# dhruvmetha/rapid-locomotion-rl

Hardware: AMD Instinct MI355X
Metric: env-steps/sec, 4096 Mini Cheetah envs, 1/2/4/8 MI355X; PPO iters/sec (higher is better)
Workload: dtype f32; 1 GPU; 4096 Mini Cheetah envs flat terrain (4096 per GPU), PPO teacher policy (BASELINE configs[1]); envs_per_gpu=4096, global_envs=4096, global_batch_env_steps_per_iter=98304, parallelism=dp1, world_size=1, policy=ActorCritic 42/18/630->12, random init; teacher PPO + student adaptation update

## Files before the change

### rapid-locomotion-rl_amd/csrc/lrl_gemm.h

```cpp
#pragma once
#include <stdint.h>

#ifdef __HIPCC__
#define LRL_GHD __host__ __device__
#else
#define LRL_GHD
#endif

namespace lrl {

enum GemmEpi : int {
  EPI_STORE = 0,
  EPI_BIAS = 1,
  EPI_BIAS_ELU = 2,
  EPI_DELU = 3,
  EPI_PARTIAL = 4,
  EPI_BIAS_TANH = 5,
  EPI_DTANH = 6,
};

struct GemmP {
  const float* A;
  const float* B;
  float* C;
  const float* bias;
  const float* aux;
  const int64_t* a_rows;
  const int64_t* b_rows;
  float* bias_part;
  int M, N, K;
  int splits, kps;
  int avec, bvec;
  int groups;
  int64_t lda, ldb, ldc, ld_aux;
  int64_t ga, gb, gc, gbias, gaux;
  int64_t part_stride;
  const uint16_t* bpl;
  int64_t bpl_ld, bpl_ps, gbp;
};

struct PlaneJob {
  const float* W;
  int64_t ldw, gsrc;
  int rows, cols, trans, groups;
  uint16_t* dst;
};
constexpr int MAX_PLANE_JOBS = 8;
LRL_GHD inline int plane_kp(const PlaneJob& j) { return ((j.trans ? j.rows : j.cols) + 15) / 16 * 16; }
LRL_GHD inline int plane_n(const PlaneJob& j) { return j.trans ? j.cols : j.rows; }
LRL_GHD inline int64_t plane_elems(const PlaneJob& j) { return 3ll * j.groups * plane_n(j) * plane_kp(j); }
int x6_planes_launch(const PlaneJob* jobs, int n, void* stream);
bool gemm_x6p_enabled();
inline void gemm_use_planes(GemmP& p, const PlaneJob& j) {
  p.bpl = j.dst;
  p.bpl_ld = plane_kp(j);
  p.gbp = (int64_t)plane_n(j) * plane_kp(j);
  p.bpl_ps = p.gbp * j.groups;
}

enum GemmLayout : int { GEMM_NT = 0, GEMM_NN = 2, GEMM_TN = 3 };

int gemm_launch(const GemmP& p, int layout, int epi, int groups, void* stream);

struct GemmJob {
  GemmP p;
  int layout, epi, groups;
};
constexpr int MAX_MULTI_JOBS = 3;
int gemm_launch_multi(const GemmJob* jobs, int n, void* stream);

enum GemmFamily : int {
  FAM_NONE = 0, FAM_X6P = 1, FAM_X6T = 2, FAM_X6 = 3, FAM_X6D = 4, FAM_GLDS = 5, FAM_GLDS32 = 6, FAM_GLDS_TN = 7,
  FAM_THIN16 = 8, FAM_THIN32 = 9, FAM_STAGED = 10,
};
constexpr int gemm_path_id(int family, int bm, int bn, bool interior) {
  return family | (bm << 8) | (bn << 16) | (interior ? 1 << 24 : 0);
}
int gemm_last_path();

int gemm_pick_splits(int M, int N, int K, int groups);

bool gemm_x6_enabled();
constexpr int X6_MIN_M = 64;

#ifdef __HIPCC__
typedef float f32x16 __attribute__((ext_vector_type(16)));
typedef short bf16x8_t __attribute__((ext_vector_type(8)));
constexpr int XBK = 16;

__device__ __forceinline__ float elu_f(float x) { return x > 0.f ? x : expm1f(x); }
__device__ __forceinline__ float tanh_f(float x) { return tanhf(x); }
__host__ __device__ constexpr bool epi_bias(int e) { return e == EPI_BIAS || e == EPI_BIAS_ELU || e == EPI_BIAS_TANH; }
__host__ __device__ constexpr bool epi_aux(int e) { return e == EPI_DELU || e == EPI_DTANH; }
template <int EPI>
__device__ __forceinline__ float epi_apply(float v, float bj, float x) {
  if constexpr (EPI == EPI_BIAS) return v + bj;
  else if constexpr (EPI == EPI_BIAS_ELU) return elu_f(v + bj);
  else if constexpr (EPI == EPI_BIAS_TANH) return tanh_f(v + bj);
  else if constexpr (EPI == EPI_DELU) return x > 0.f ? v : v * (x + 1.f);
  else if constexpr (EPI == EPI_DTANH) return v * (1.f - x * x);
  else return v;
}

__device__ __forceinline__ uint32_t x6_hi_pair(uint32_t u0, uint32_t u1) {
  return __builtin_amdgcn_perm(u1, u0, 0x07060302u);
}
__device__ __forceinline__ void x6_split2(float x0, float x1, uint32_t& h, uint32_t& m, uint32_t& l) {
  uint32_t u0 = __float_as_uint(x0), u1 = __float_as_uint(x1);
  h = x6_hi_pair(u0, u1);
  float r0 = x0 - __uint_as_float(u0 & 0xffff0000u), r1 = x1 - __uint_as_float(u1 & 0xffff0000u);
  u0 = __float_as_uint(r0);
  u1 = __float_as_uint(r1);
  m = x6_hi_pair(u0, u1);
  r0 = r0 - __uint_as_float(u0 & 0xffff0000u);
  r1 = r1 - __uint_as_float(u1 & 0xffff0000u);
  l = x6_hi_pair(__float_as_uint(r0), __float_as_uint(r1));
}
__device__ __forceinline__ int x6_off(int r, int c) { return r * XBK + 8 * (c ^ ((r >> 3) & 1)); }

__device__ __forceinline__ f32x16 x6_mma(const bf16x8_t (&a)[3], const bf16x8_t (&b)[3], f32x16 c) {
  c = __builtin_amdgcn_mfma_f32_32x32x16_bf16(a[2], b[0], c, 0, 0, 0);
  c = __builtin_amdgcn_mfma_f32_32x32x16_bf16(a[1], b[1], c, 0, 0, 0);
  c = __builtin_amdgcn_mfma_f32_32x32x16_bf16(a[0], b[2], c, 0, 0, 0);
  c = __builtin_amdgcn_mfma_f32_32x32x16_bf16(a[1], b[0], c, 0, 0, 0);
  c = __builtin_amdgcn_mfma_f32_32x32x16_bf16(a[0], b[1], c, 0, 0, 0);
  c = __builtin_amdgcn_mfma_f32_32x32x16_bf16(a[0], b[0], c, 0, 0, 0);
  return c;
}
#endif

}
```

### rapid-locomotion-rl_amd/csrc/lrl_ppo.hip

```cpp
#include <hip/hip_runtime.h>
#include <math.h>
#include <stdint.h>
#include <stdlib.h>
#include <string.h>

#include <algorithm>
#include <initializer_list>
#include <mutex>
#include <vector>

#include "../../include/lrl.h"
#include "../../include/lrl_philox.h"
#include "lrl_gemm.h"
#include "lrl_launch.h"

namespace lrl {

constexpr float LOG_SQRT_2PI = 0.91893853320467274178f;
constexpr int HEAD_ROWS = 32;
constexpr int HEAD_THREADS = 256;
constexpr int HEAD_W = 128;
constexpr int MAX_ACT = 16;
constexpr int HEAD_NA = 12;
constexpr int MAX_LAT = 32;

__device__ __forceinline__ float delu(float h) { return h > 0.f ? 1.f : h + 1.f; }

constexpr int PREP_R = 4;
__global__ void ppo_prep_kernel(const float* __restrict__ obs, const int64_t* __restrict__ rows, int B, int no,
                                int xs, float* __restrict__ X) {
  const int64_t i = (int64_t)blockIdx.x * blockDim.x + threadIdx.x;
  const int64_t ng = ((int64_t)B + PREP_R - 1) / PREP_R;
  if (i >= ng * xs) return;
  const int g = (int)(i / xs), c = (int)(i - (int64_t)g * xs);
  int64_t src[PREP_R];
  float v[PREP_R];
#pragma unroll
  for (int u = 0; u < PREP_R; ++u) {
    const int b = g * PREP_R + u;
    src[u] = b < B ? (rows ? rows[b] : (int64_t)b) : -1;
  }
#pragma unroll
  for (int u = 0; u < PREP_R; ++u) v[u] = (c < no && src[u] >= 0) ? obs[src[u] * no + c] : 0.f;
#pragma unroll
  for (int u = 0; u < PREP_R; ++u) {
    const int b = g * PREP_R + u;
    if (b < B) X[(int64_t)b * xs + c] = v[u];
  }
}

inline unsigned prep_blocks(int64_t rows, int xs) {
  return (unsigned)((((rows + PREP_R - 1) / PREP_R) * xs + 255) / 256);
}

struct HeadArgs {
  const float* h3;
  float* dh3;
  const float *w4a, *b4a, *w4c, *b4c, *stdv;
  const float *actions, *old_mu, *old_sigma, *tv, *ret, *adv, *old_logp;
  const int64_t* rows;
  int B, na;
  float clip, ent_coef, vcoef;
  int clipped_value;
  float* part;
  int part_len;
};

__host__ __device__ constexpr int hp_w4a(int) { return 0; }
__host__ __device__ constexpr int hp_b4a(int na) { return na * HEAD_W; }
__host__ __device__ constexpr int hp_w4c(int na) { return na * HEAD_W + na; }
__host__ __device__ constexpr int hp_b4c(int na) { return na * HEAD_W + na + HEAD_W; }
__host__ __device__ constexpr int hp_std(int na) { return na * HEAD_W + na + HEAD_W + 1; }
__host__ __device__ constexpr int hp_kl(int na) { return na * HEAD_W + na + HEAD_W + 1 + na; }
__host__ __device__ constexpr int hp_len(int na) { return hp_kl(na) + 3; }

template <int NA, bool TANH>
__global__ __launch_bounds__(HEAD_THREADS) void ppo_head_kernel(HeadArgs a) {
  constexpr int HP = 2 * HEAD_W + 4;
  constexpr int NAP = (NA + 3) / 4 * 4;
  static_assert(NA <= 16 && HEAD_W % 16 == 0, "float4 rows");
  constexpr int NG = (HEAD_ROWS * NA + HEAD_THREADS - 1) / HEAD_THREADS;
  __shared__ __attribute__((aligned(16))) float H[HEAD_ROWS][HP];
  __shared__ __attribute__((aligned(16))) float W4[NA + 1][HEAD_W];
  __shared__ float MU[HEAD_ROWS][NA + 1];
  __shared__ float VP[HEAD_ROWS][8];
  __shared__ __attribute__((aligned(16))) float LP[HEAD_ROWS][NAP];
  __shared__ float KT[HEAD_ROWS][NA];
  __shared__ float DR[HEAD_ROWS][2];
  __shared__ float SC[HEAD_ROWS][3];
  __shared__ float SD[3][NA];
  __shared__ float GA[3][HEAD_ROWS][NA];
  __shared__ float GR[4][HEAD_ROWS];
  __shared__ int64_t RW[HEAD_ROWS];
  const int t = threadIdx.x;
  const int r0 = blockIdx.x * HEAD_ROWS;
  const int nrows = min(HEAD_ROWS, a.B - r0);
  if (t < HEAD_ROWS) RW[t] = t < nrows ? a.rows[r0 + t] : a.rows[r0];
  if (t < NA) {
    const float sd = a.stdv[t];
    SD[0][t] = sd;
    SD[1][t] = logf(sd);
    SD[2][t] = 1.f / (sd * sd);
  }
  {
    constexpr int NV = HEAD_ROWS * 2 * HEAD_W / 4 / HEAD_THREADS;
    float4 v[NV];
#pragma unroll
    for (int u = 0; u < NV; ++u) {
      const int i = t + u * HEAD_THREADS, r = i / (HEAD_W / 2), c = 4 * (i % (HEAD_W / 2));
      v[u] = r < nrows ? *reinterpret_cast<const float4*>(a.h3 + (int64_t)(r0 + r) * (2 * HEAD_W) + c)
                       : make_float4(0.f, 0.f, 0.f, 0.f);
    }
#pragma unroll
    for (int u = 0; u < NV; ++u) {
      const int i = t + u * HEAD_THREADS, r = i / (HEAD_W / 2), c = 4 * (i % (HEAD_W / 2));
      *reinterpret_cast<float4*>(&H[r][c]) = v[u];
    }
  }
  for (int i = t; i < (NA + 1) * HEAD_W; i += HEAD_THREADS) {
    const int j = i / HEAD_W, k = i - j * HEAD_W;
    W4[j][k] = j < NA ? a.w4a[j * HEAD_W + k] : a.w4c[k];
  }
  __syncthreads();
  float ga[3][NG], gr = 0.f;
#pragma unroll
  for (int u = 0; u < NG; ++u) {
    const int i = t + u * HEAD_THREADS;
    const int r = i / NA, j = i - r * NA;
    const bool ok = i < HEAD_ROWS * NA;
    const int64_t o = RW[ok ? r : 0] * NA + j;
    ga[0][u] = ok ? a.actions[o] : 0.f;
    ga[1][u] = ok ? a.old_mu[o] : 0.f;
    ga[2][u] = ok ? a.old_sigma[o] : 1.f;
  }
  if (t < 4 * HEAD_ROWS) {
    const int q = t / HEAD_ROWS, r = t - q * HEAD_ROWS;
    const float* src = q == 0 ? a.adv : q == 1 ? a.old_logp : q == 2 ? a.tv : a.ret;
    gr = src[RW[r]];
  }
  {
    const int r = t & (HEAD_ROWS - 1), q = t / HEAD_ROWS;
    const float4* hr = reinterpret_cast<const float4*>(&H[r][0]);
    auto dot4 = [](float s, float4 h, float4 w) {
      s = fmaf(h.x, w.x, s);
      s = fmaf(h.y, w.y, s);
      s = fmaf(h.z, w.z, s);
      return fmaf(h.w, w.w, s);
    };
    for (int j = q; j < NA; j += 8) {
      const float4* wr = reinterpret_cast<const float4*>(&W4[j][0]);
      float s = 0.f;
#pragma unroll 8
      for (int k4 = 0; k4 < HEAD_W / 4; ++k4) s = dot4(s, hr[k4], wr[k4]);
      MU[r][j] = s + a.b4a[j];
    }
// ... 714 lines not shown
      else oa_layer<1>(L);
      __syncthreads();
      FA_PROF(5 + l)
    }
    const int64_t so = (int64_t)a.store_row * a.n;
    if (grp == 0) {
      for (int e = t; e < NA * HEAD_W; e += OA_THREADS) HW[e] = w[nt.w4a + e];
      __syncthreads();
      for (int e = t; e < OA_R * NA; e += OA_THREADS) {
        const int r = e & (OA_R - 1), j = e / OA_R;
        float s = 0.f;
        for (int k = 0; k < HEAD_W; ++k) s = fmaf(H3[r * OA_H3P + k], HW[j * HEAD_W + k], s);
        MU[r * 16 + j] = s + w[nt.b4a + j];
      }
      __syncthreads();
      FA_PROF(8)
      for (int i = t; i < nrows * NA; i += OA_THREADS) {
        const int r = i / NA, j = i - r * NA, g = r0 + r;
        const float m = MU[r * 16 + j], sd = w[nt.std_off + j];
        float act;
        MU[r * 16 + j] = act_draw(a.eps, a.row_offset, a.seed, a.counter, g, j, NA, m, sd, act);
        a.actions[(int64_t)g * NA + j] = act;
        if (a.mu) a.mu[(int64_t)g * NA + j] = m;
        if (a.do_store) {
          const int64_t o = (so + g) * NA + j;
          a.store.actions[o] = act;
          a.store.mu[o] = m;
          a.store.sigma[o] = sd;
        }
      }
      __syncthreads();
      if (t < nrows) {
        const int g = r0 + t;
        float lp = 0.f;
        for (int j = 0; j < NA; ++j) lp += MU[t * 16 + j];
        if (a.logp) a.logp[g] = lp;
        if (a.do_store) a.store.logp[so + g] = lp;
      }
    } else {
      for (int e = t; e < HEAD_W; e += OA_THREADS) HW[e] = w[nt.w4c + e];
      __syncthreads();
      for (int e = t; e < OA_R * 16; e += OA_THREADS) {
        const int r = e & (OA_R - 1), q = e / OA_R;
        float s = 0.f;
        for (int k = q * (HEAD_W / 16); k < (q + 1) * (HEAD_W / 16); ++k) s = fmaf(H3[r * OA_H3P + k], HW[k], s);
        VP[r * 16 + q] = s;
      }
      __syncthreads();
      FA_PROF(8)
      if (t < nrows) {
        const int g = r0 + t;
        float vs[16];
#pragma unroll
        for (int q = 0; q < 16; ++q) vs[q] = VP[t * 16 + q];
#pragma unroll
        for (int wd = 8; wd >= 1; wd /= 2)
#pragma unroll
          for (int q = 0; q < wd; ++q) vs[q] = vs[2 * q] + vs[2 * q + 1];
        const float v = vs[0] + w[nt.b4c];
        if (a.values) a.values[g] = v;
        if (a.do_store) a.store.values[so + g] = v;
      }
    }
    FA_PROF(9)
    if (a.do_store) {
      const int64_t b = so + r0;
      if (grp == 0) copy_rows<OA_THREADS>(a.obs + (int64_t)r0 * no, no, a.store.obs + b * no, no, nrows, no, t);
      else copy_rows<OA_THREADS>(a.priv + (int64_t)r0 * np, np, a.store.priv + b * np, np, nrows, np, t);
      if (a.hist && a.store.hist) {
        const int hd = a.store.hist_dim, ld = a.store.hist_ld > hd ? a.store.hist_ld : hd;
        const int h0 = grp * (OA_R / 2), hn = min(nrows, h0 + OA_R / 2) - h0;
        if (hn > 0) copy_rows<OA_THREADS>(a.hist + (int64_t)(r0 + h0) * hd, hd, a.store.hist + (b + h0) * ld, ld, hn, hd, t);
      }
    }
    FA_PROF(10)
  }
}

struct AdaptHeadArgs {
  const float* hd2;
  int ldh;
  const float* tgt;
  int ldt;
  float* dhd2;
  const float *w, *b;
  int B, H, L;
  float* part;
  int part_len;
};

template <int CH, int CL>
__global__ __launch_bounds__(HEAD_THREADS) void adapt_head_kernel(AdaptHeadArgs a) {
  const int H = CH ? CH : a.H, L = CL ? CL : a.L;
  __shared__ float HS[HEAD_ROWS][MAX_LAT + 1];
  __shared__ float DP[HEAD_ROWS][MAX_LAT + 1];
  __shared__ float WS[MAX_LAT][MAX_LAT + 1];
  __shared__ float TG[HEAD_ROWS][MAX_LAT + 1];
  __shared__ float ERR[HEAD_ROWS];
  const int t = threadIdx.x;
  const int r0 = blockIdx.x * HEAD_ROWS;
  const int nrows = min(HEAD_ROWS, a.B - r0);
  for (int i = t; i < HEAD_ROWS * H; i += HEAD_THREADS) {
    const int r = i / H, c = i - r * H;
    HS[r][c] = r < nrows ? a.hd2[(int64_t)(r0 + r) * a.ldh + c] : 0.f;
  }
  for (int i = t; i < L * H; i += HEAD_THREADS) WS[i / H][i % H] = a.w[i];
  for (int i = t; i < HEAD_ROWS * L; i += HEAD_THREADS) {
    const int r = i / L, j = i - r * L;
    TG[r][j] = r < nrows ? a.tgt[(int64_t)(r0 + r) * a.ldt + j] : 0.f;
  }
  __syncthreads();
  const float scale = 2.f / ((float)a.B * (float)L);
  for (int i = t; i < HEAD_ROWS * L; i += HEAD_THREADS) {
    const int r = i / L, j = i - r * L;
    float d = 0.f;
    if (r < nrows) {
      float s = 0.f;
      for (int k = 0; k < H; ++k) s = fmaf(HS[r][k], WS[j][k], s);
      const float pred = s + a.b[j];
      d = pred - TG[r][j];
    }
    TG[r][j] = d * d;
    DP[r][j] = scale * d;
  }
  __syncthreads();
  if (t < HEAD_ROWS) {
    float e = 0.f;
    for (int j = 0; j < L; ++j) e += TG[t][j];
    ERR[t] = e;
  }
  __syncthreads();
  float* P = a.part + (int64_t)blockIdx.x * a.part_len;
  for (int i = t; i < nrows * H; i += HEAD_THREADS) {
    const int r = i / H, k = i - r * H;
    float s = 0.f;
    for (int j = 0; j < L; ++j) s = fmaf(DP[r][j], WS[j][k], s);
    a.dhd2[(int64_t)(r0 + r) * a.ldh + k] = s * delu(HS[r][k]);
  }
  const int nr = CH ? HEAD_ROWS : nrows;
  for (int i = t; i < L * H; i += HEAD_THREADS) {
    const int j = i / H, k = i - j * H;
    float s = 0.f;
    for (int r = 0; r < nr; ++r) s = fmaf(DP[r][j], HS[r][k], s);
    P[i] = s;
  }
  if (t < L) {
    float s = 0.f;
    for (int r = 0; r < nr; ++r) s += DP[r][t];
    P[L * H + t] = s;
  } else if (t == 64) {
    float s = 0.f;
    for (int r = 0; r < nr; ++r) s += ERR[r];
    P[L * H + L] = s;
  }
}

struct Seg {
  const float* src;
  float* dst;
  int64_t len, stride;
  int parts;
  float scale;
  int lpg;
  int blk0, nblk;
};
constexpr int MAX_SEGS = 24;
struct SegList {
  Seg s[MAX_SEGS];
  int n;
};

__global__ __launch_bounds__(256) void seg_reduce_kernel(SegList L) {
  int si = 0;
  while (si + 1 < L.n && (int)blockIdx.x >= L.s[si + 1].blk0) ++si;
  const Seg& sg = L.s[si];
  const int lpg = sg.lpg, pg = 1 << lpg, E = 256 >> lpg;
  const int e = threadIdx.x & (E - 1), g = threadIdx.x >> (8 - lpg);
  __shared__ float red[256];
  for (int64_t base = (int64_t)(blockIdx.x - sg.blk0) * E; base < sg.len; base += (int64_t)sg.nblk * E) {
    const int64_t i = base + e;
    float acc = 0.f;
    if (i < sg.len) {
      const float* p = sg.src + i;
      int q = g;
      for (; q + 7 * pg < sg.parts; q += 8 * pg) {
        float v[8];
#pragma unroll
        for (int u = 0; u < 8; ++u) v[u] = __builtin_nontemporal_load(p + (int64_t)(q + u * pg) * sg.stride);
#pragma unroll
        for (int u = 0; u < 8; ++u) acc += v[u];
      }
      for (; q < sg.parts; q += pg) acc += p[(int64_t)q * sg.stride];
    }
    if (pg == 1) {
      if (i < sg.len) sg.dst[i] = acc * sg.scale;
      continue;
    }
    red[threadIdx.x] = acc;
    __syncthreads();
    if (g == 0 && i < sg.len) {
      float t = 0.f;
      for (int k = 0; k < pg; ++k) t += red[k * E + e];
      sg.dst[i] = t * sg.scale;
    }
    __syncthreads();
  }
}

constexpr int NORM_BLOCKS = 256;
__global__ void sumsq_kernel(const float* __restrict__ g, int64_t n, double* __restrict__ part) {
  double s = 0.0;
  for (int64_t i = (int64_t)blockIdx.x * blockDim.x + threadIdx.x; i < n; i += (int64_t)gridDim.x * blockDim.x) {
    const double x = g[i];
    s += x * x;
  }
  for (int off = 32; off > 0; off >>= 1) s += __shfl_down(s, off, 64);
  __shared__ double red[4];
  if ((threadIdx.x & 63) == 0) red[threadIdx.x >> 6] = s;
  __syncthreads();
  if (threadIdx.x == 0) part[blockIdx.x] = (red[0] + red[1]) + (red[2] + red[3]);
}

__global__ void ppo_finalize_kernel(const double* __restrict__ part, int nparts, const float* __restrict__ kl_slot,
                                    float grad_scale, float max_norm, float desired_kl, int adaptive, double bc1,
                                    float inv_B, lrl_ppo_ctrl* ctrl) {
  __shared__ double red[64];
  double s = 0.0;
  for (int i = threadIdx.x; i < nparts; i += 64) s += part[i];
  red[threadIdx.x] = s;
  __syncthreads();
  if (threadIdx.x != 0) return;
  double tot = 0.0;
  for (int i = 0; i < 64; ++i) tot += red[i];
  const float total_norm = (float)sqrt(tot) * grad_scale;
  float clip = max_norm / (total_norm + 1e-6f);
  clip = fminf(clip, 1.f);
  double lr = ctrl->lr;
  const float kl = kl_slot[0] * grad_scale;
  if (adaptive) {
    const double k = (double)kl;
    if (k > (double)desired_kl * 2.0) lr = fmax(1e-5, lr / 1.5);
    else if (k < (double)desired_kl / 2.0 && k > 0.0) lr = fmin(1e-2, lr * 1.5);
  }
  ctrl->lr = lr;
  ctrl->mb[3] = kl;
  ctrl->clip_scale = clip;
  ctrl->total_norm = total_norm;
  ctrl->step_size = (float)(lr / bc1);
  ctrl->loss_sum[0] += (double)ctrl->mb[0];
  ctrl->loss_sum[1] += (double)ctrl->mb[1];
}

__global__ void adam_kernel(float* __restrict__ p, const float* __restrict__ g, float* __restrict__ m,
                            float* __restrict__ v, int64_t n, float grad_scale, const lrl_ppo_ctrl* __restrict__ ctrl,
                            float step_size_host, float one_minus_b1, float b2, float one_minus_b2, float bc2_sqrt,
                            float eps, lrl_ppo_ctrl* acc_ctrl) {
  const float clip = ctrl ? ctrl->clip_scale : 1.f;
  const float step = ctrl ? ctrl->step_size : step_size_host;
  for (int64_t i = (int64_t)blockIdx.x * blockDim.x + threadIdx.x; i < n; i += (int64_t)gridDim.x * blockDim.x) {
    float gi = g[i] * grad_scale;
    gi = gi * clip;
    float mi = m[i];
    mi = mi + one_minus_b1 * (gi - mi);
    float vi = v[i] * b2;
    vi = vi + one_minus_b2 * gi * gi;
    m[i] = mi;
    v[i] = vi;
    const float denom = sqrtf(vi) / bc2_sqrt + eps;
    p[i] = p[i] + (-step) * (mi / denom);
  }
  if (acc_ctrl && blockIdx.x == 0 && threadIdx.x == 0) acc_ctrl->loss_sum[2] += (double)acc_ctrl->mb[2];
}

__global__ void pad_cols_kernel(const float* __restrict__ W, int rows, int h, int hp, float* __restrict__ Wp) {
  const int64_t n = (int64_t)rows * hp;
  for (int64_t i = (int64_t)blockIdx.x * blockDim.x + threadIdx.x; i < n; i += (int64_t)gridDim.x * blockDim.x) {
    const int r = (int)(i / hp), c = (int)(i - (int64_t)r * hp);
    Wp[i] = c < h ? W[(int64_t)r * h + c] : 0.f;
  }
}


static int xs_of(const lrl_ppo_net& n) {
  if (n.plain) return (n.num_obs + 15) / 16 * 16;
  const int nx = n.num_obs + n.latent;
  return nx <= 64 ? 64 : (nx + 15) / 16 * 16;
}
constexpr int LATS = 32;
constexpr int HD2S = 32;
static int hist_pad(int h) { return (h + 15) / 16 * 16; }

enum MainPlane { PL_W1, PL_W2, PL_W3, PL_E2, PL_W2T, PL_W3T, PL_E2T, PL_MAIN };
constexpr int PL_FWD = PL_E2 + 1;
enum AdaptPlane { PL_D1, PL_AE2, PL_D2T, PL_ADAPT };

struct Layer {
  int64_t w, b;
  int out, in;
  int64_t ldw;
  int kf;
  int groups;
  int fwd, bwd;
};
static Layer layer(int64_t w, int64_t b, int out, int in, int groups = 1, int fwd = -1, int bwd = -1) {
  return Layer{w, b, out, in, in, in, groups, fwd, bwd};
}
// ... 556 lines not shown
  return hipGetLastError() == hipSuccess ? 0 : lrl_set_error(LRL_E_HIP, "lrl_ppo_act: launch failed");
}

extern "C" int64_t lrl_ppo_act_student_workspace_bytes(const lrl_ppo_net* net, int32_t n) {
  if (check_net(net) || net->plain || n <= 0) return -1;
  return make_student_plan(*net, n, nullptr).bytes;
}

extern "C" int32_t lrl_ppo_act_student(const lrl_ppo_net* net, const float* params, const float* obs,
                                       const float* hist, int32_t hist_ld, int32_t n, float* mean, float* latent,
                                       void* workspace, void* stream) {
  if (int rc = check_net(net)) return rc;
  if (net->plain) return lrl_set_error(LRL_E_INVALID, "lrl_ppo_act_student: a plain net has no adaptation module");
  if (!params || !obs || !hist || !mean || !workspace || n <= 0)
    return lrl_set_error(LRL_E_INVALID, "lrl_ppo_act_student: null argument or n <= 0");
  const lrl_ppo_net& nt = *net;
  const int hld = hist_ld ? hist_ld : nt.num_hist;
  if (hld < nt.num_hist) return lrl_set_error(LRL_E_INVALID, "lrl_ppo_act_student: hist_ld < num_hist");
  Plan P = make_student_plan(nt, n, static_cast<char*>(workspace));
  hipStream_t st = static_cast<hipStream_t>(stream);
  G g{st, params, n};
  const Net L = layers_of(nt, true);
  const Buf lat = cols_from(P.xa, nt.num_obs);
  prep_x(nt, obs, nullptr, n, P.xa, st);
  adaptation_l1_forward(g, L.ad[0], In{hist, hld}, nullptr, P);
  g.forward(L.ad[1], P.hd1, nullptr, P.hd2, true);
  g.forward(L.ad[2], P.hd2, nullptr, lat, false);
  body_forward(g, L.body, P);
  g.forward(L.mean, P.h3, nullptr, Buf{mean, nt.num_actions}, false);
  if (g.rc) return lrl_set_error(g.rc, "lrl_ppo_act_student: GEMM launch failed");
  if (latent &&
      hipMemcpy2DAsync(latent, (size_t)nt.latent * 4, lat.p, (size_t)lat.ld * 4, (size_t)nt.latent * 4, n,
                       hipMemcpyDeviceToDevice, st) != hipSuccess)
    return lrl_set_error(LRL_E_HIP, "lrl_ppo_act_student: latent copy failed");
  return hipGetLastError() == hipSuccess ? 0 : lrl_set_error(LRL_E_HIP, "lrl_ppo_act_student: launch failed");
}

extern "C" int64_t lrl_ppo_workspace_bytes(const lrl_ppo_net* net, int32_t batch) {
  if (check_net(net) || batch <= 0) return -1;
  return make_plan(*net, batch, nullptr).bytes;
}

extern "C" int32_t lrl_ppo_forward_backward(const lrl_ppo_net* net, const float* params, float* grads,
                                            const lrl_ppo_batch* bt, const lrl_ppo_hparams* hp, void* workspace,
                                            lrl_ppo_ctrl* ctrl, void* stream) {
  if (int rc = check_net(net)) return rc;
  if (!bt || !hp || !params || !grads || !workspace || !ctrl || bt->batch <= 0)
    return lrl_set_error(LRL_E_INVALID, "lrl_ppo_forward_backward: null argument");
  const lrl_ppo_net& n = *net;
  const int B = bt->batch;
  const bool full = !n.plain;
  Plan P = make_plan(n, B, static_cast<char*>(workspace));
  hipStream_t st = static_cast<hipStream_t>(stream);
  G g{st, params, B, P.part, P.part + P.part_floats};
  g.tanh_act = n.plain;
  const Net net_l = layers_of(n);
  const Layer(&enc)[3] = net_l.enc;
  const Layer(&body)[3] = net_l.body;
  PlaneJob pj[PL_MAIN];
  if (full) {
    main_plane_jobs(n, params, P.wpl, pj);
    if (int rc = split_planes(pj, PL_MAIN, gemm_x6p_enabled(), st))
      return lrl_set_error(rc, "lrl_ppo_forward_backward: planes launch failed");
    g.with(pj);
  }
  const In priv{bt->priv, n.num_priv};
  prep_x(n, bt->obs, bt->rows, B, P.xa, st);
  if (full) encoder_forward(g, enc, priv, bt->rows, P, cols_from(P.xa, n.num_obs));
  body_forward(g, body, P);
  if (g.rc) return lrl_set_error(g.rc, "lrl_ppo_forward_backward: forward GEMM launch failed");
  SegList L{};
  launch_loss_head(n, params, grads, bt, hp, ctrl, P, g.part, L, st);
  g.backward_data(body[2], P.dh3, P.dh2, P.h2);
  g.backward_data(body[1], P.dh2, P.dh1, P.h1);
  if (full) g.backward_data(net_l.dlat, P.dh1, P.dlat, In{});
  enum { DWE3, DHE2, DWE2, DHE1, DWE1, DW3, DW2, DW1, NJOBS };
  GemmJob jobs[NJOBS];
  const int first = full ? 0 : DW3;
  g.collect(jobs, first, NJOBS);
  if (full) {
    g.weight_grad(enc[2], P.dlat, P.he2, nullptr, grads, L);
    g.backward_data(enc[2], P.dlat, P.dhe2, P.he2);
    g.weight_grad(enc[1], P.dhe2, P.he1, nullptr, grads, L);
    g.backward_data(enc[1], P.dhe2, P.dhe1, P.he1);
    g.weight_grad(enc[0], P.dhe1, priv, bt->rows, grads, L);
  }
  g.weight_grad(body[2], P.dh3, P.h2, nullptr, grads, L);
  g.weight_grad(body[1], P.dh2, P.h1, nullptr, grads, L);
  g.weight_grad(body[0], P.dh1, P.xa, nullptr, grads, L);
  int rc = g.rc ? g.rc : (g.njobs == NJOBS ? 0 : LRL_E_INVALID);
  if (rc) return lrl_set_error(rc, "lrl_ppo_forward_backward: backward GEMM launch failed");
  struct Set { int n, i[MAX_MULTI_JOBS]; };
  Set sets[NJOBS];
  int ns = 0;
  const int mode = full ? bwd_multi_mode() : 0;
  if (mode == 0) {
    for (int i = first; i < NJOBS; ++i) sets[ns++] = Set{1, {i}};
  } else if (g_timer.on) {
    sets[ns++] = Set{3, {DWE3, DHE2, DW3}};
    sets[ns++] = Set{2, {DWE2, DHE1}};
    sets[ns++] = Set{1, {DW2}};
    sets[ns++] = Set{2, {DWE1, DW1}};
  } else {
    static const int hosts[3][3] = {{DW3, DW1, DW2}, {DW3, DW2, DW1}, {DW2, DW1, DW3}};
    const int* host = hosts[mode - 1];
    sets[ns++] = Set{3, {DWE3, DHE2, host[0]}};
    sets[ns++] = Set{3, {DWE2, DHE1, host[1]}};
    sets[ns++] = Set{2, {DWE1, host[2]}};
  }
  Fork* fk = mode == 0 && full ? fork_for_device(st) : nullptr;
  if (fk && (hipEventRecord(fk->go, st) != hipSuccess || hipStreamWaitEvent(fk->st, fk->go, 0) != hipSuccess))
    return lrl_set_error(LRL_E_HIP, "lrl_ppo_forward_backward: stream fork failed");
  for (int s = 0; s < ns && !rc; ++s) {
    const int lead = sets[s].i[0];
    const bool timed = full && sets[s].n == 1 && lead == DW2;
    if (timed) timer_begin(st);
    rc = launch_jobs(jobs, sets[s].i, sets[s].n, fk && lead < DW3 ? fk->st : st);
    if (timed) timer_end(st);
    if (fk && lead == DWE1 && hipEventRecord(fk->done, fk->st) != hipSuccess)
      return lrl_set_error(LRL_E_HIP, "lrl_ppo_forward_backward: stream fork failed");
  }
  if (fk && hipStreamWaitEvent(st, fk->done, 0) != hipSuccess)
    return lrl_set_error(LRL_E_HIP, "lrl_ppo_forward_backward: stream join failed");
  if (rc) return lrl_set_error(rc, "lrl_ppo_forward_backward: backward GEMM launch failed");
  launch_seg(L, st);
  return hipGetLastError() == hipSuccess ? 0 : lrl_set_error(LRL_E_HIP, "lrl_ppo_forward_backward: launch failed");
}

extern "C" int32_t lrl_ppo_optimizer_step(const lrl_ppo_net* net, float* params, const float* grads, float* exp_avg,
                                          float* exp_avg_sq, int64_t step, float grad_scale,
                                          const lrl_ppo_hparams* hp, void* workspace, lrl_ppo_ctrl* ctrl,
                                          void* stream) {
  if (int rc = check_net(net)) return rc;
  if (!params || !grads || !exp_avg || !exp_avg_sq || !hp || !workspace || !ctrl || step < 1)
    return lrl_set_error(LRL_E_INVALID, "lrl_ppo_optimizer_step: bad argument");
  const lrl_ppo_net& n = *net;
  hipStream_t st = static_cast<hipStream_t>(stream);
  double* norm_part = static_cast<double*>(workspace);
  const int64_t len = n.main_end - n.main_begin;
  hipLaunchKernelGGL(sumsq_kernel, dim3(NORM_BLOCKS), dim3(256), 0, st, grads + n.main_begin, len, norm_part);
  const double bc1 = 1.0 - pow((double)hp->beta1, (double)step);
  const double bc2 = 1.0 - pow((double)hp->beta2, (double)step);
  hipLaunchKernelGGL(ppo_finalize_kernel, dim3(1), dim3(64), 0, st, norm_part, NORM_BLOCKS,
                     grads + n.kl_slot, grad_scale, hp->max_grad_norm, hp->desired_kl, hp->adaptive_schedule, bc1,
                     0.f, ctrl);
  const int blocks = (int)std::min<int64_t>((len + 255) / 256, 2048);
  hipLaunchKernelGGL(adam_kernel, dim3(blocks), dim3(256), 0, st, params + n.main_begin, grads + n.main_begin,
                     exp_avg + n.main_begin, exp_avg_sq + n.main_begin, len, grad_scale, ctrl, 0.f,
                     (float)(1.0 - (double)hp->beta1), hp->beta2, (float)(1.0 - (double)hp->beta2), (float)sqrt(bc2),
                     hp->eps, (lrl_ppo_ctrl*)nullptr);
  return hipGetLastError() == hipSuccess ? 0 : lrl_set_error(LRL_E_HIP, "lrl_ppo_optimizer_step: launch failed");
}

extern "C" int32_t lrl_ppo_adaptation_forward_backward(const lrl_ppo_net* net, const float* params,
                                                       const float* enc_params, float* grads, const lrl_ppo_batch* bt,
                                                       void* workspace, lrl_ppo_ctrl* ctrl, void* stream) {
  if (int rc = check_net(net)) return rc;
  if (net->plain)
    return lrl_set_error(LRL_E_INVALID, "lrl_ppo_adaptation_forward_backward: a plain net has no adaptation module");
  if (!bt || !params || !grads || !workspace || !ctrl || bt->batch <= 0)
    return lrl_set_error(LRL_E_INVALID, "lrl_ppo_adaptation_forward_backward: null argument");
  const lrl_ppo_net& n = *net;
  const int B = bt->batch;
  const int hld = bt->hist_ld ? bt->hist_ld : n.num_hist;
  if (hld < n.num_hist) return lrl_set_error(LRL_E_INVALID, "lrl_ppo_adaptation: hist_ld < num_hist");
  Plan P = make_plan(n, B, static_cast<char*>(workspace));
  hipStream_t st = static_cast<hipStream_t>(stream);
  G g{st, params, B, P.part, P.part + P.part_floats};
  const Net net_l = layers_of(n);
  const Layer(&ad)[3] = net_l.ad;
  const float* we = enc_params ? enc_params : params;
  PlaneJob pj[PL_ADAPT];
  adapt_plane_jobs(n, params, we, P.wpl, pj);
  if (int rc = split_planes(pj, PL_ADAPT, gemm_x6p_enabled(), st))
    return lrl_set_error(rc, "lrl_ppo_adaptation: planes launch failed");
  g.with(pj);
  g.w = we;
  encoder_forward(g, net_l.tgt, In{bt->priv, n.num_priv}, bt->rows, P, P.tgt);
  g.w = params;
  const In hist{bt->hist, hld};
  adaptation_l1_forward(g, ad[0], hist, bt->rows, P);
  g.forward(ad[1], P.hd1, nullptr, P.hd2, true);
  if (g.rc) return lrl_set_error(g.rc, "lrl_ppo_adaptation: forward GEMM launch failed");
  SegList L{};
  float*& part = g.part;
  const int hb = (B + HEAD_ROWS - 1) / HEAD_ROWS;
  AdaptHeadArgs aa{};
  aa.hd2 = P.hd2.p; aa.ldh = HD2S; aa.tgt = P.tgt.p; aa.ldt = LATS; aa.dhd2 = P.dhd2.p; aa.w = params + n.d3w;
  aa.b = params + n.d3b;
  aa.B = B; aa.H = n.ad_h1; aa.L = n.latent; aa.part = part; aa.part_len = n.latent * n.ad_h1 + n.latent + 1;
  if (aa.H == 32 && aa.L == 18)
    hipLaunchKernelGGL((adapt_head_kernel<32, 18>), dim3(hb), dim3(HEAD_THREADS), 0, st, aa);
  else
    hipLaunchKernelGGL((adapt_head_kernel<0, 0>), dim3(hb), dim3(HEAD_THREADS), 0, st, aa);
  {
    const int64_t pl = aa.part_len;
    L.s[L.n++] = Seg{part, grads + n.d3w, (int64_t)n.latent * n.ad_h1, pl, hb, 1.f};
    L.s[L.n++] = Seg{part + n.latent * n.ad_h1, grads + n.d3b, n.latent, pl, hb, 1.f};
    L.s[L.n++] = Seg{part + n.latent * n.ad_h1 + n.latent, &ctrl->mb[2], 1, pl, hb,
                     1.f / ((float)B * (float)n.latent)};
    part += ((hb * pl + 63) / 64) * 64;
  }
  g.weight_grad(ad[1], P.dhd2, P.hd1, nullptr, grads, L);
  g.backward_data(ad[1], P.dhd2, P.dhd1, P.hd1);
  g.weight_grad(ad[0], P.dhd1, hist, bt->rows, grads, L);
  if (g.rc) return lrl_set_error(g.rc, "lrl_ppo_adaptation: backward GEMM launch failed");
  launch_seg(L, st);
  return hipGetLastError() == hipSuccess ? 0 : lrl_set_error(LRL_E_HIP, "lrl_ppo_adaptation: launch failed");
}

extern "C" int32_t lrl_ppo_adaptation_step(const lrl_ppo_net* net, float* params, const float* grads, float* exp_avg,
                                           float* exp_avg_sq, int64_t step, double lr, float grad_scale,
                                           const lrl_ppo_hparams* hp, lrl_ppo_ctrl* ctrl, void* stream) {
  if (int rc = check_net(net)) return rc;
  if (net->plain) return lrl_set_error(LRL_E_INVALID, "lrl_ppo_adaptation_step: a plain net has no adaptation module");
  if (!params || !grads || !exp_avg || !exp_avg_sq || !hp || step < 1)
    return lrl_set_error(LRL_E_INVALID, "lrl_ppo_adaptation_step: bad argument");
  const lrl_ppo_net& n = *net;
  hipStream_t st = static_cast<hipStream_t>(stream);
  const double bc1 = 1.0 - pow((double)hp->beta1, (double)step);
  const double bc2 = 1.0 - pow((double)hp->beta2, (double)step);
  const int64_t len = n.adapt_end - n.adapt_begin;
  const int blocks = (int)std::min<int64_t>((len + 255) / 256, 2048);
  hipLaunchKernelGGL(adam_kernel, dim3(blocks), dim3(256), 0, st, params + n.adapt_begin, grads + n.adapt_begin,
                     exp_avg + n.adapt_begin, exp_avg_sq + n.adapt_begin, len, grad_scale,
                     (const lrl_ppo_ctrl*)nullptr, (float)(lr / bc1), (float)(1.0 - (double)hp->beta1), hp->beta2,
                     (float)(1.0 - (double)hp->beta2), (float)sqrt(bc2), hp->eps, ctrl);
  return hipGetLastError() == hipSuccess ? 0 : lrl_set_error(LRL_E_HIP, "lrl_ppo_adaptation_step: launch failed");
}

static int use_test_planes(GemmP& p, int layout, int groups, float* workspace, int64_t workspace_floats,
                           hipStream_t st) {
  PlaneJob j = plane_job(p.B, p.ldb, layout, p.N, p.K, groups, p.gb);
  j.dst = reinterpret_cast<uint16_t*>(workspace);
  if (!workspace || plane_elems(j) > 2 * workspace_floats)
    return lrl_set_error(LRL_E_INVALID, "lrl_gemm_f32(_ex): workspace too small for the planes");
  if (int rc = x6_planes_launch(&j, 1, st)) return lrl_set_error(rc, "lrl_gemm_f32(_ex): planes launch failed");
  gemm_use_planes(p, j);
  return 0;
}

extern "C" int32_t lrl_gemm_f32(int32_t layout, int32_t epi, int32_t M, int32_t N, int32_t K, const float* A,
                                int64_t lda, const float* B, int64_t ldb, float* C, int64_t ldc, const float* bias,
                                const float* aux, int64_t ld_aux, const int64_t* rows, float* workspace,
                                int64_t workspace_floats, void* stream) {
  hipStream_t st = static_cast<hipStream_t>(stream);
  if ((epi == EPI_BIAS_TANH && (layout & 0xff) != GEMM_NT) || (epi == EPI_DTANH && (layout & 0xff) != GEMM_NN))
    return lrl_set_error(LRL_E_INVALID, "lrl_gemm_f32: epi 5 is an NT epilogue, epi 6 an NN one");
  if (epi == EPI_DTANH && !aux) return lrl_set_error(LRL_E_INVALID, "lrl_gemm_f32: epi 6 needs aux");
  if (layout == GEMM_TN) {
    if (ldc != N) return lrl_set_error(LRL_E_INVALID, "lrl_gemm_f32: TN needs ldc == N");
    int splits = 0;
    if (const char* e = getenv("LRL_GEMM_SPLITS")) splits = std::max(atoi(e), 0);
    SplitK k;
    float* part = workspace;
    if (!splitk_job(M, N, K, 1, splits, In{A, lda}, 0, In{B, ldb}, 0, rows, C, const_cast<float*>(bias), part,
                    workspace + workspace_floats, k))
      return lrl_set_error(LRL_E_INVALID, "lrl_gemm_f32: workspace too small");
    if (int rc = gemm_launch(k.p, GEMM_TN, EPI_PARTIAL, 1, st)) return lrl_set_error(rc, "lrl_gemm_f32: launch failed");
    SegList L{};
    L.s[L.n++] = k.s[0];
    if (bias) L.s[L.n++] = k.s[1];
    launch_seg(L, st);
    return hipGetLastError() == hipSuccess ? 0 : lrl_set_error(LRL_E_HIP, "lrl_gemm_f32: launch failed");
  }
  GemmP p{};
  p.A = A; p.lda = lda; p.B = B; p.ldb = ldb; p.C = C; p.ldc = ldc; p.bias = bias; p.aux = aux; p.ld_aux = ld_aux;
  p.M = M; p.N = N; p.K = K; p.splits = 1;
  p.a_rows = rows;
  if (layout & 0x100) {
    layout &= 0xff;
    if (layout != GEMM_NT && layout != GEMM_NN) return lrl_set_error(LRL_E_INVALID, "lrl_gemm_f32: planes need NT / NN");
    if (int rc = use_test_planes(p, layout, 1, workspace, workspace_floats, st)) return rc;
    int rc = gemm_launch(p, layout, epi, 1, st);
    if (rc) return lrl_set_error(rc, "lrl_gemm_f32: launch failure");
    return (gemm_last_path() & 0xff) == FAM_X6P
               ? 0
               : lrl_set_error(LRL_E_INVALID, "lrl_gemm_f32: shape not eligible for the x6p kernel");
  }
  int rc = gemm_launch(p, layout, epi, 1, st);
  return rc ? lrl_set_error(rc, "lrl_gemm_f32: bad layout/epilogue or launch failure") : 0;
}

static int32_t desc_job(const lrl_gemm_desc* d, GemmJob& job, SplitK& k) {
  if (!d || !d->A || !d->B || !d->C || d->M <= 0 || d->N <= 0 || d->K <= 0 || d->groups <= 0 || d->splits < 0)
    return lrl_set_error(LRL_E_INVALID, "lrl_gemm_f32_ex: bad argument");
  const int layout = d->layout, epi = d->epi, groups = d->groups, M = d->M, N = d->N, K = d->K;
  if (d->path_out) *d->path_out = 0;
  if (layout == GEMM_TN) {
    if (epi != EPI_PARTIAL || d->planes) return lrl_set_error(LRL_E_INVALID, "lrl_gemm_f32_ex: TN is epi 4, no planes");
    if (d->ldc != N) return lrl_set_error(LRL_E_INVALID, "lrl_gemm_f32_ex: TN needs ldc == N");
    if (d->splits) {
      const int kps = ((K + d->splits - 1) / d->splits + 15) / 16 * 16;
      if ((int64_t)(d->splits - 1) * kps >= K) return lrl_set_error(LRL_E_INVALID, "lrl_gemm_f32_ex: a split would be empty");
    }
    float* part = d->workspace;
    if (!d->workspace || !splitk_job(M, N, K, groups, d->splits, In{d->A, d->lda}, d->ga, In{d->B, d->ldb}, d->gb,
                                     d->rows, d->C, d->bias, part, d->workspace + d->workspace_floats, k))
      return lrl_set_error(LRL_E_INVALID, "lrl_gemm_f32_ex: workspace too small");
    job =GemmJob{k.p, layout, epi, groups};
    return 0;
  }
  if (layout != GEMM_NT && layout != GEMM_NN) return lrl_set_error(LRL_E_INVALID, "lrl_gemm_f32_ex: layout is 0, 2 or 3");
  if (d->splits > 1 || epi == EPI_PARTIAL) return lrl_set_error(LRL_E_INVALID, "lrl_gemm_f32_ex: NT / NN are not split");
  if ((epi == EPI_BIAS_TANH && layout != GEMM_NT) || (epi == EPI_DTANH && layout != GEMM_NN))
    return lrl_set_error(LRL_E_INVALID, "lrl_gemm_f32_ex: epi 5 is an NT epilogue, epi 6 an NN one");
  if ((epi == EPI_DELU || epi == EPI_DTANH) && !d->aux) return lrl_set_error(LRL_E_INVALID, "lrl_gemm_f32_ex: epi 3 / 6 need aux");
  if ((epi == EPI_BIAS || epi == EPI_BIAS_ELU || epi == EPI_BIAS_TANH) && !d->bias)
    return lrl_set_error(LRL_E_INVALID, "lrl_gemm_f32_ex: epi 1 / 2 / 5 need bias");
  GemmP p{};
  p.A = d->A; p.lda = d->lda; p.B = d->B; p.ldb = d->ldb; p.aux = d->aux; p.ld_aux = d->ld_aux;
  p.M = M; p.N = N; p.K = K; p.splits = 1;
  p.ga = d->ga; p.gb = d->gb; p.gaux = d->gaux;
  p.C = d->C; p.ldc = d->ldc; p.gc = d->gc; p.bias = d->bias; p.gbias = d->gbias; p.a_rows = d->rows;
  k.p = p;
  job = GemmJob{p, layout, epi, groups};
  return 0;
}
static void desc_reduce(const lrl_gemm_desc* d, const GemmJob& job, const SplitK& k, SegList& L) {
  if (job.layout != GEMM_TN) return;
  L.s[L.n++] = k.s[0];
  if (d->bias) L.s[L.n++] = k.s[1];
}

extern "C" int32_t lrl_gemm_f32_ex(const lrl_gemm_desc* d, void* stream) {
  GemmJob job;
  SplitK k;
  if (int32_t rc = desc_job(d, job, k)) return rc;
  hipStream_t st = static_cast<hipStream_t>(stream);
  GemmP& p = job.p;
  const int layout = job.layout, epi = job.epi, groups = job.groups;
  if (layout == GEMM_TN) {
    if (int rc = gemm_launch(p, GEMM_TN, EPI_PARTIAL, groups, st)) return lrl_set_error(rc, "lrl_gemm_f32_ex: launch failed");
    SegList L{};
    desc_reduce(d, job, k, L);
    launch_seg(L, st);
  } else {
    if (d->planes)
      if (int rc = use_test_planes(p, layout, groups, d->workspace, d->workspace_floats, st)) return rc;
    if (int rc = gemm_launch(p, layout, epi, groups, st))
      return lrl_set_error(rc, "lrl_gemm_f32_ex: bad layout/epilogue or launch failure");
    if (d->planes && (gemm_last_path() & 0xff) != FAM_X6P)
      return lrl_set_error(LRL_E_INVALID, "lrl_gemm_f32_ex: shape not eligible for the x6p kernel");
  }
  if (d->path_out) *d->path_out = gemm_last_path();
  if (d->splits_out) *d->splits_out = k.p.splits;
  return hipGetLastError() == hipSuccess ? 0 : lrl_set_error(LRL_E_HIP, "lrl_gemm_f32_ex: launch failed");
}

extern "C" int32_t lrl_gemm_f32_multi(const lrl_gemm_desc* d, int32_t n, void* stream) {
  if (!d || n < 2 || n > MAX_MULTI_JOBS) return lrl_set_error(LRL_E_INVALID, "lrl_gemm_f32_multi: 2 or 3 descriptors");
  hipStream_t st = static_cast<hipStream_t>(stream);
  GemmJob jobs[MAX_MULTI_JOBS];
  SplitK ks[MAX_MULTI_JOBS];
  for (int i = 0; i < n; ++i) {
    if (d[i].planes) return lrl_set_error(LRL_E_INVALID, "lrl_gemm_f32_multi: no planes");
    if (int32_t rc = desc_job(&d[i], jobs[i], ks[i])) return rc;
// ... 32 lines not shown
```

Measured before the change: 4.128 million env-steps/s.

## Fuse adaptation layer-2 forward, head, and layer-2 backward-data into one kernel

Adds an adapt_tail_kernel that, per 32-row block, computes the second adaptation layer (256->32, bias+ELU) with split-bf16 MFMA, then the latent head loss and gradients, then the backward-data GEMM back to 256 columns with the ELU derivative. When shapes match (256/32/18, aligned params, x6 enabled), this replaces a forward GEMM, the head kernel and a backward-data GEMM launch. It removes the intermediate hd2 round trip and two launches, but the fused kernel runs the MFMA work in a single wave for the forward part. It can be disabled with an environment variable. The adaptation update is a small part of the PPO iteration.

```diff
diff --git a/rapid-locomotion-rl_amd/csrc/lrl_gemm.h b/rapid-locomotion-rl_amd/csrc/lrl_gemm.h
--- a/rapid-locomotion-rl_amd/csrc/lrl_gemm.h
+++ b/rapid-locomotion-rl_amd/csrc/lrl_gemm.h
@@ -116,6 +116,16 @@
   r1 = r1 - __uint_as_float(u1 & 0xffff0000u);
   l = x6_hi_pair(__float_as_uint(r0), __float_as_uint(r1));
 }
+__device__ __forceinline__ void x6_split8(const float (&x)[8], bf16x8_t (&o)[3]) {
+  uint32_t hh[4], mm[4], ll[4];
+#pragma unroll
+  for (int e = 0; e < 4; ++e) x6_split2(x[2 * e], x[2 * e + 1], hh[e], mm[e], ll[e]);
+  uint4 vh = make_uint4(hh[0], hh[1], hh[2], hh[3]), vm = make_uint4(mm[0], mm[1], mm[2], mm[3]),
+        vl = make_uint4(ll[0], ll[1], ll[2], ll[3]);
+  o[0] = *reinterpret_cast<bf16x8_t*>(&vh);
+  o[1] = *reinterpret_cast<bf16x8_t*>(&vm);
+  o[2] = *reinterpret_cast<bf16x8_t*>(&vl);
+}
 __device__ __forceinline__ int x6_off(int r, int c) { return r * XBK + 8 * (c ^ ((r >> 3) & 1)); }
 
 __device__ __forceinline__ f32x16 x6_mma(const bf16x8_t (&a)[3], const bf16x8_t (&b)[3], f32x16 c) {
diff --git a/rapid-locomotion-rl_amd/csrc/lrl_ppo.hip b/rapid-locomotion-rl_amd/csrc/lrl_ppo.hip
--- a/rapid-locomotion-rl_amd/csrc/lrl_ppo.hip
+++ b/rapid-locomotion-rl_amd/csrc/lrl_ppo.hip
@@ -1,6 +1,7 @@
 #include <hip/hip_runtime.h>
 #include <math.h>
 #include <stdint.h>
+#include <stdio.h>
 #include <stdlib.h>
 #include <string.h>
 
@@ -1021,6 +1022,176 @@
     float s = 0.f;
     for (int r = 0; r < nr; ++r) s += ERR[r];
     P[L * H + L] = s;
+  }
+}
+
+constexpr int AT_K = 256, AT_H = 32, AT_L = 18;
+constexpr int AT_XP = AT_K + 4;
+constexpr int AT_DP = AT_H + 4;
+struct AdaptTailArgs {
+  AdaptHeadArgs head;
+  const float* hd1;
+  float* dhd1;
+  const float *w2, *b2;
+};
+
+__global__ __launch_bounds__(HEAD_THREADS, 3) void adapt_tail_kernel(AdaptTailArgs ta) {
+  constexpr int H = AT_H, L = AT_L;
+  const AdaptHeadArgs& a = ta.head;
+  __shared__ __attribute__((aligned(16))) float X1[HEAD_ROWS][AT_XP];
+  __shared__ __attribute__((aligned(16))) float DH[HEAD_ROWS][AT_DP];
+  __shared__ float HS[HEAD_ROWS][MAX_LAT + 1];
+  __shared__ float DP[HEAD_ROWS][L + 1];
+  __shared__ float WS[L][MAX_LAT + 1];
+  __shared__ float TG[HEAD_ROWS][L + 1];
+  __shared__ float ERR[HEAD_ROWS];
+  const int t = threadIdx.x, lane = t & 63, wv = t >> 6, li = lane & 31, h = lane >> 5;
+  const int r0 = blockIdx.x * HEAD_ROWS;
+  const int nrows = min(HEAD_ROWS, a.B - r0);
+  constexpr int NX = HEAD_ROWS * AT_K / 4 / HEAD_THREADS;
+  constexpr int PF = 4;
+  float4 xv[NX];
+#pragma unroll
+  for (int u = 0; u < NX; ++u) {
+    const int i = t + HEAD_THREADS * u, r = i / (AT_K / 4), c = i % (AT_K / 4);
+    xv[u] = r < nrows ? *reinterpret_cast<const float4*>(ta.hd1 + (int64_t)(r0 + r) * AT_K + 4 * c)
+                      : make_float4(0.f, 0.f, 0.f, 0.f);
+  }
+  const float* wrow = ta.w2 + li * AT_K + 8 * h;
+  float4 bq[PF][2];
+  if (wv == 0) {
+#pragma unroll
+    for (int s = 0; s < PF; ++s) {
+      bq[s][0] = *reinterpret_cast<const float4*>(wrow + XBK * s);
+      bq[s][1] = *reinterpret_cast<const float4*>(wrow + XBK * s + 4);
+    }
+  }
+  for (int i = t; i < L * H; i += HEAD_THREADS) WS[i / H][i % H] = a.w[i];
+  for (int i = t; i < HEAD_ROWS * L; i += HEAD_THREADS) {
+    const int r = i / L, j = i - r * L;
+    TG[r][j] = r < nrows ? a.tgt[(int64_t)(r0 + r) * a.ldt + j] : 0.f;
+  }
+#pragma unroll
+  for (int u = 0; u < NX; ++u) {
+    const int i = t + HEAD_THREADS * u, r = i / (AT_K / 4), c = i % (AT_K / 4);
+    *reinterpret_cast<float4*>(&X1[r][4 * c]) = xv[u];
+  }
+  __syncthreads();
+  if (wv == 0) {
+    f32x16 acc;
+#pragma unroll
+    for (int r = 0; r < 16; ++r) acc[r] = 0.f;
+#pragma unroll
+    for (int s = 0; s < AT_K / XBK; ++s) {
+      const float4 b0 = bq[s % PF][0], b1 = bq[s % PF][1];
+      if (s + PF < AT_K / XBK) {
+        bq[s % PF][0] = *reinterpret_cast<const float4*>(wrow + XBK * (s + PF));
+        bq[s % PF][1] = *reinterpret_cast<const float4*>(wrow + XBK * (s + PF) + 4);
+      }
+      const float4 x0 = *reinterpret_cast<const float4*>(&X1[li][XBK * s + 8 * h]);
+      const float4 x1 = *reinterpret_cast<const float4*>(&X1[li][XBK * s + 8 * h + 4]);
+      const float xa[8] = {x0.x, x0.y, x0.z, x0.w, x1.x, x1.y, x1.z, x1.w};
+      const float xb[8] = {b0.x, b0.y, b0.z, b0.w, b1.x, b1.y, b1.z, b1.w};
+      bf16x8_t af[3], bf[3];
+      x6_split8(xa, af);
+      x6_split8(xb, bf);
+      acc = x6_mma(af, bf, acc);
+    }
+    const float bj = ta.b2[li];
+#pragma unroll
+    for (int q = 0; q < 4; ++q)
+#pragma unroll
+      for (int r = 0; r < 4; ++r) {
+        const int row = 8 * q + 4 * h + r;
+        HS[row][li] = row < nrows ? epi_apply<EPI_BIAS_ELU>(acc[4 * q + r], bj, 0.f) : 0.f;
+      }
+  }
+  float wb[2][2][8];
+#pragma unroll
+  for (int s = 0; s < 2; ++s)
+#pragma unroll
+    for (int j = 0; j < 2; ++j)
+#pragma unroll
+      for (int e = 0; e < 8; ++e) wb[s][j][e] = ta.w2[(XBK * s + 8 * h + e) * AT_K + 64 * wv + 32 * j + li];
+  __syncthreads();
+  const float scale = 2.f / ((float)a.B * (float)L);
+  for (int i = t; i < HEAD_ROWS * L; i += HEAD_THREADS) {
+    const int r = i / L, j = i - r * L;
+    float d = 0.f;
+    if (r < nrows) {
+      float s = 0.f;
+      for (int k = 0; k < H; ++k) s = fmaf(HS[r][k], WS[j][k], s);
+      const float pred = s + a.b[j];
+      d = pred - TG[r][j];
+    }
+    TG[r][j] = d * d;
+    DP[r][j] = scale * d;
+  }
+  __syncthreads();
+  if (t < HEAD_ROWS) {
+    float e = 0.f;
+    for (int j = 0; j < L; ++j) e += TG[t][j];
+    ERR[t] = e;
+  }
+  __syncthreads();
+  float* P = a.part + (int64_t)blockIdx.x * a.part_len;
+  for (int i = t; i < HEAD_ROWS * H; i += HEAD_THREADS) {
+    const int r = i / H, k = i - r * H;
+    float v = 0.f;
+    if (r < nrows) {
+      float s = 0.f;
+      for (int j = 0; j < L; ++j) s = fmaf(DP[r][j], WS[j][k], s);
+      v = s * delu(HS[r][k]);
+      a.dhd2[(int64_t)(r0 + r) * a.ldh + k] = v;
+    }
+    DH[r][k] = v;
+  }
+  for (int i = t; i < L * H; i += HEAD_THREADS) {
+    const int j = i / H, k = i - j * H;
+    float s = 0.f;
+    for (int r = 0; r < HEAD_ROWS; ++r) s = fmaf(DP[r][j], HS[r][k], s);
+    P[i] = s;
+  }
+  if (t < L) {
+    float s = 0.f;
+    for (int r = 0; r < HEAD_ROWS; ++r) s += DP[r][t];
+    P[L * H + t] = s;
+  } else if (t == 64) {
+    float s = 0.f;
+    for (int r = 0; r < HEAD_ROWS; ++r) s += ERR[r];
+    P[L * H + L] = s;
+  }
+  __syncthreads();
+  f32x16 dac[2];
+#pragma unroll
+  for (int j = 0; j < 2; ++j)
+#pragma unroll
+    for (int r = 0; r < 16; ++r) dac[j][r] = 0.f;
+#pragma unroll
+  for (int s = 0; s < H / XBK; ++s) {
+    const float4 x0 = *reinterpret_cast<const float4*>(&DH[li][XBK * s + 8 * h]);
+    const float4 x1 = *reinterpret_cast<const float4*>(&DH[li][XBK * s + 8 * h + 4]);
+    const float xa[8] = {x0.x, x0.y, x0.z, x0.w, x1.x, x1.y, x1.z, x1.w};
+    bf16x8_t af[3];
+    x6_split8(xa, af);
+#pragma unroll
+    for (int j = 0; j < 2; ++j) {
+      bf16x8_t bf[3];
+      x6_split8(wb[s][j], bf);
+      dac[j] = x6_mma(af, bf, dac[j]);
+    }
+  }
+#pragma unroll
+  for (int j = 0; j < 2; ++j) {
+    const int col = 64 * wv + 32 * j + li;
+#pragma unroll
+    for (int q = 0; q < 4; ++q)
+#pragma unroll
+      for (int r = 0; r < 4; ++r) {
+        const int row = 8 * q + 4 * h + r;
+        if (row < nrows)
+          ta.dhd1[(int64_t)(r0 + row) * AT_K + col] = epi_apply<EPI_DELU>(dac[j][4 * q + r], 0.f, X1[row][col]);
+      }
   }
 }
 
@@ -1883,6 +2054,14 @@
   return hipGetLastError() == hipSuccess ? 0 : lrl_set_error(LRL_E_HIP, "lrl_ppo_optimizer_step: launch failed");
 }
 
+static bool adapt_tail_fits(const lrl_ppo_net& n, const float* params, int rows) {
+  const char* e = getenv("LRL_ADAPT_TAIL");
+  if (e && e[0] == '0') return false;
+  if (rows < X6_MIN_M || (int64_t)rows * AT_K >= (int64_t(1) << 31) || !gemm_x6_enabled()) return false;
+  if (n.ad_h0 != AT_K || n.ad_h1 != AT_H || n.latent != AT_L) return false;
+  return (reinterpret_cast<uintptr_t>(params + n.d2w) & 15) == 0;
+}
+
 extern "C" int32_t lrl_ppo_adaptation_forward_backward(const lrl_ppo_net* net, const float* params,
                                                        const float* enc_params, float* grads, const lrl_ppo_batch* bt,
                                                        void* workspace, lrl_ppo_ctrl* ctrl, void* stream) {
@@ -1911,7 +2090,8 @@
   g.w = params;
   const In hist{bt->hist, hld};
   adaptation_l1_forward(g, ad[0], hist, bt->rows, P);
-  g.forward(ad[1], P.hd1, nullptr, P.hd2, true);
+  const bool tail = adapt_tail_fits(n, params, B);
+  if (!tail) g.forward(ad[1], P.hd1, nullptr, P.hd2, true);
   if (g.rc) return lrl_set_error(g.rc, "lrl_ppo_adaptation: forward GEMM launch failed");
   SegList L{};
   float*& part = g.part;
@@ -1920,7 +2100,12 @@
   aa.hd2 = P.hd2.p; aa.ldh = HD2S; aa.tgt = P.tgt.p; aa.ldt = LATS; aa.dhd2 = P.dhd2.p; aa.w = params + n.d3w;
   aa.b = params + n.d3b;
   aa.B = B; aa.H = n.ad_h1; aa.L = n.latent; aa.part = part; aa.part_len = n.latent * n.ad_h1 + n.latent + 1;
-  if (aa.H == 32 && aa.L == 18)
+  if (tail) {
+    static const bool trace = getenv("LRL_GEMM_TRACE") != nullptr;
+    if (trace) fprintf(stderr, "adapt_tail M=%d workgroups=%d\n", B, hb);
+    AdaptTailArgs ta{aa, P.hd1.p, P.dhd1.p, params + n.d2w, params + n.d2b};
+    hipLaunchKernelGGL(adapt_tail_kernel, dim3(hb), dim3(HEAD_THREADS), 0, st, ta);
+  } else if (aa.H == 32 && aa.L == 18)
     hipLaunchKernelGGL((adapt_head_kernel<32, 18>), dim3(hb), dim3(HEAD_THREADS), 0, st, aa);
   else
     hipLaunchKernelGGL((adapt_head_kernel<0, 0>), dim3(hb), dim3(HEAD_THREADS), 0, st, aa);
@@ -1933,7 +2118,7 @@
     part += ((hb * pl + 63) / 64) * 64;
   }
   g.weight_grad(ad[1], P.dhd2, P.hd1, nullptr, grads, L);
-  g.backward_data(ad[1], P.dhd2, P.dhd1, P.hd1);
+  if (!tail) g.backward_data(ad[1], P.dhd2, P.dhd1, P.hd1);
   g.weight_grad(ad[0], P.dhd1, hist, bt->rows, grads, L);
   if (g.rc) return lrl_set_error(g.rc, "lrl_ppo_adaptation: backward GEMM launch failed");
   launch_seg(L, st);
```

Result: no change. 4.157 million env-steps/s (median of 6 runs) (+0.7%).
